# azuxmioy/Render-In-Between

Hardware: AMD Instinct MI355X
Metric: rendered frames/sec at 512x512 (generator forward + blend, device-resident) (higher is better)
Workload: dtype f32

## Files before the change

### include/rib.h

```cpp
#ifndef RIB_H
#define RIB_H

#include <stddef.h>
#include <stdint.h>

#ifdef __cplusplus
extern "C" {
#endif

typedef struct rib_handle rib_handle;

typedef enum {
  RIB_OK = 0,
  RIB_ERR_INVALID = -1,
  RIB_ERR_UNSUPPORTED = -2,
  RIB_ERR_STATE = -3,
  RIB_ERR_MISSING = -4,
  RIB_ERR_HIP = -5,
  RIB_ERR_WORKSPACE = -6
} rib_status;

typedef struct {
  int32_t label_nc;
  int32_t image_nc;
// ... 104 lines not shown
int rib_num_launches(rib_handle* h, int B, int H, int W);

int rib_num_variants(void);
int rib_variant_info(int idx, int geom[12]);
int rib_set_choice(rib_handle* h, int B, int H, int W, const char* op_name, int variant_idx, int ksplit);
int rib_time_op(rib_handle* h, int B, int H, int W, const char* op_name, const float* label,
                const float* img_fake, const float* img_prev, float* img, float* mask, void* workspace,
                size_t workspace_bytes, int iters, void* hip_stream, double* usec);

int rib_set_graph_replay(rib_handle* h, int enable);
int rib_graph_stats(rib_handle* h, int64_t* captures, int64_t* replays);

int rib_set_plan_batch(rib_handle* h, int n);
int rib_get_plan_batch(const rib_handle* h);

const char* rib_build_info(void);

int rib_debug_conv_weight(rib_handle* h, const char* conv_name, float* w_oihw, float* bias);
int rib_debug_spade_weight(rib_handle* h, const char* conv_name, float* w_2c_by_cond, float* bias_2c);
int rib_debug_launch_info(rib_handle* h, int B, int H, int W, int idx, char* buf, size_t buflen);

#ifdef __cplusplus
}
#endif
#endif
```

### render-in-between_amd/_native.py

```python
from __future__ import annotations

import ctypes as C
import os

_HERE = os.path.dirname(os.path.abspath(__file__))
LIB_PATH = os.environ.get("RIB_LIBRARY") or os.path.join(_HERE, "csrc", "librib.so")

KC_NAMES = ("igemm", "spade", "stats", "pool", "eltwise", "pack", "conv_aux")


class RibConfig(C.Structure):
    _fields_ = [(n, C.c_int32) for n in (
        "label_nc", "image_nc", "num_filters", "max_num_filters", "num_layers", "num_down_img",
        "emb_filters", "emb_max_filters", "emb_down", "mask_filters", "mask_max_filters",
        "mask_down", "mask_res_blocks")]


class RibError(RuntimeError):
    def __init__(self, code, msg):
        super().__init__("rib error %d: %s" % (code, msg))
        self.code = code


_lib = None
# ... 54 lines not shown
    "rib_forward_flops": (C.c_int, [C.c_void_p, C.c_int, C.c_int, C.c_int, C.POINTER(C.c_double)]),
    "rib_num_launches": (C.c_int, [C.c_void_p, C.c_int, C.c_int, C.c_int]),
    "rib_num_variants": (C.c_int, []),
    "rib_variant_info": (C.c_int, [C.c_int, C.POINTER(C.c_int)]),
    "rib_set_choice": (C.c_int, [C.c_void_p, C.c_int, C.c_int, C.c_int, C.c_char_p, C.c_int, C.c_int]),
    "rib_time_op": (C.c_int, [C.c_void_p, C.c_int, C.c_int, C.c_int, C.c_char_p] + [C.c_void_p] * 6
                    + [C.c_size_t, C.c_int, C.c_void_p, C.POINTER(C.c_double)]),
    "rib_debug_conv_weight": (C.c_int, [C.c_void_p, C.c_char_p, C.c_void_p, C.c_void_p]),
    "rib_debug_spade_weight": (C.c_int, [C.c_void_p, C.c_char_p, C.c_void_p, C.c_void_p]),
    "rib_debug_launch_info": (C.c_int, [C.c_void_p, C.c_int, C.c_int, C.c_int, C.c_int, C.c_char_p, C.c_size_t]),
    "rib_build_info": (C.c_char_p, []),
    "rib_set_graph_replay": (C.c_int, [C.c_void_p, C.c_int]),
    "rib_graph_stats": (C.c_int, [C.c_void_p, C.POINTER(C.c_int64), C.POINTER(C.c_int64)]),
    "rib_set_plan_batch": (C.c_int, [C.c_void_p, C.c_int]),
    "rib_get_plan_batch": (C.c_int, [C.c_void_p]),
}


def lib():
    global _lib
    if _lib is None:
        if not os.path.exists(LIB_PATH):
            raise RuntimeError(
                "native library %s is missing: build it with "
                "`python render-in-between_amd/csrc/build.py` (there is no CPU fallback)" % LIB_PATH)
        import torch
        L = C.CDLL(LIB_PATH)
        for name, (res, args) in SIGNATURES.items():
            fn = getattr(L, name)
            fn.restype = res
# ... 17 lines not shown
```

### render-in-between_amd/csrc/kernels.hip.h

```cpp
#pragma once
#include "igemm.hip.h"

namespace rib {

struct GemmDmaParams {
  const float* A; const float* B; float* C;
  int M, N, K, lda, ldc;
  size_t sA, sB, sC;
  int modB;
  int K2; unsigned long long kmask;
};

typedef uint32_t u32x4 __attribute__((ext_vector_type(4)));
__device__ __forceinline__ void split3_bf16(const float4 p, const float4 q, bf16x8& hi, bf16x8& mid, bf16x8& lo) {
  const float x[8] = {p.x, p.y, p.z, p.w, q.x, q.y, q.z, q.w};
  u32x4 h, m, l;
#pragma unroll
  for (int i = 0; i < 4; ++i) {
    const uint32_t u0 = __float_as_uint(x[2 * i]), u1 = __float_as_uint(x[2 * i + 1]);
    h[i] = __builtin_amdgcn_perm(u1, u0, 0x07060302u);
    const float r0 = x[2 * i] - __uint_as_float(u0 & 0xffff0000u), r1 = x[2 * i + 1] - __uint_as_float(u1 & 0xffff0000u);
    const uint32_t v0 = __float_as_uint(r0), v1 = __float_as_uint(r1);
    m[i] = __builtin_amdgcn_perm(v1, v0, 0x07060302u);
    const float s0 = r0 - __uint_as_float(v0 & 0xffff0000u), s1 = r1 - __uint_as_float(v1 & 0xffff0000u);
// ... 294 lines not shown
    for (int k = 0; k < 4; ++k) { t1 += red[(k * 64 + j) * 2]; t2 += red[(k * 64 + j) * 2 + 1]; }
    float sc, sh;
    scale_shift_of(t1, t2, s.inv_count, s.gamma ? s.gamma[c0 + j] : 1.f, s.beta ? s.beta[c0 + j] : 0.f, sc, sh);
    s_sc[j] = sc; s_sh[j] = sh;
  }
  __syncthreads();
}

enum { WSRC_PLAIN = 0, WSRC_SPADE = 1, WSRC_JOIN = 2 };
struct WinoInParams {
  const float* x; int H, W, xC, Cin;
  const float* pro_scale; const float* pro_shift; int pro_ld, pro_lrelu;
  StatSrc st;
  float* v; int tilesY, tilesX;
  int nslices, ublocks;
  int x_ups; const float* slab; int slab_ld, col0; const float* sbias;
  const float* x2; const float* xres; float* o; const float* pro2_scale; const float* pro2_shift; StatSrc st2;
  int ldv;
  int nslices2, Cin2, xC2, x2_ups, lrelu2, pro2_ld;
  const float* slab2; int slab2_ld, col0_2; const float* sbias2;
};
__device__ __forceinline__ WinoInParams wino_second(const WinoInParams& p) {
  WinoInParams q = p;
  q.x = p.x2; q.xC = p.xC2; q.Cin = p.Cin2; q.x_ups = p.x2_ups; q.pro_lrelu = p.lrelu2;
  q.pro_scale = p.pro2_scale; q.pro_shift = p.pro2_shift; q.pro_ld = p.pro2_ld; q.st = p.st2;
  q.slab = p.slab2; q.slab_ld = p.slab2_ld; q.col0 = p.col0_2; q.sbias = p.sbias2;
  q.x2 = nullptr; q.v = p.v + p.Cin;
  return q;
}

// ... 66 lines not shown
                    spade_mod1(r.a.z, k.sc.z, k.sh.z, r.b.z, k.bg.z, r.c.z, k.bb.z), spade_mod1(r.a.w, k.sc.w, k.sh.w, r.b.w, k.bg.w, r.c.w, k.bb.w));
    if (p.pro_lrelu) w = lrelu4(w);
  } else if constexpr (MODE == WSRC_JOIN) {
    w = make_float4(w.x * k.sc.x + k.sh.x, w.y * k.sc.y + k.sh.y, w.z * k.sc.z + k.sh.z, w.w * k.sc.w + k.sh.w);
    if (p.x2) { w.x += r.b.x * k.sc2.x + k.sh2.x; w.y += r.b.y * k.sc2.y + k.sh2.y; w.z += r.b.z * k.sc2.z + k.sh2.z; w.w += r.b.w * k.sc2.w + k.sh2.w; }
    else { w.x += r.b.x; w.y += r.b.y; w.z += r.b.z; w.w += r.b.w; }
  } else {
    if (k.aff) w = make_float4(w.x * k.sc.x + k.sh.x, w.y * k.sc.y + k.sh.y, w.z * k.sc.z + k.sh.z, w.w * k.sc.w + k.sh.w);
    if (p.pro_lrelu) w = lrelu4(w);
  }
  return w;
}

#define RIB_F4_SUB(a, b) make_float4((a).x - (b).x, (a).y - (b).y, (a).z - (b).z, (a).w - (b).w)
#define RIB_F4_ADD(a, b) make_float4((a).x + (b).x, (a).y + (b).y, (a).z + (b).z, (a).w + (b).w)

template <int MODE, bool SC>
__device__ __forceinline__ void wino_in_slice(const WinoInParams& p, int slice, int ub, double* red, float* s_sc, float* s_sh) {
  const int c4n = p.Cin / 4;
  const int n = blockIdx.y;
  const int c4 = slice * 16 + (threadIdx.x & 15);
  const bool cok = c4 < c4n;
  const int ntiles = p.tilesY * p.tilesX;
  constexpr int NR = SC ? 2 : 4, Q0 = SC ? 1 : 0, Q1 = SC ? 3 : 4;
  WinoConsts<MODE> kc;
  wino_in_consts<MODE>(p, n, slice, c4, cok, red, s_sc, s_sh, kc);
  if (!cok) return;
  for (int u = ub * 16 + (threadIdx.x >> 4); u < ntiles * NR; u += p.ublocks * 16) {
    const int r = SC ? 1 + (u & 1) : u & 3, tile = SC ? u >> 1 : u >> 2;
    const int ty = tile / p.tilesX, tx = tile % p.tilesX;
// ... 13 lines not shown
      float4 v[2];
#pragma unroll
      for (int a = 0; a < 2; ++a) {
        const int iy = 2 * ty - 1 + (a ? ib : ia), ix = 2 * tx - 1 + q;
        const bool inb = iy >= 0 && iy < p.H && ix >= 0 && ix < p.W;
        float4 w = wino_value<MODE>(p, kc, d[a][q]);
        if constexpr (MODE == WSRC_JOIN) {
          if (r == 1 && (q == 1 || q == 2) && inb) *reinterpret_cast<float4*>(p.o + (((size_t)n * p.H + iy) * p.W + ix) * p.xC + c4 * 4) = w;
        }
        if (!inb) w = make_float4(0.f, 0.f, 0.f, 0.f);
        v[a] = w;
      }
      t[q] = make_float4(v[0].x + sg * v[1].x, v[0].y + sg * v[1].y, v[0].z + sg * v[1].z, v[0].w + sg * v[1].w);
    }
    const size_t plane = (size_t)ntiles * p.ldv;
    float* vb = p.v + (size_t)n * 16 * plane + (size_t)tile * p.ldv + c4 * 4;
    if constexpr (!SC) *reinterpret_cast<float4*>(vb + (size_t)(r * 4 + 0) * plane) = RIB_F4_SUB(t[0], t[2]);
    *reinterpret_cast<float4*>(vb + (size_t)(r * 4 + 1) * plane) = RIB_F4_ADD(t[1], t[2]);
    *reinterpret_cast<float4*>(vb + (size_t)(r * 4 + 2) * plane) = RIB_F4_SUB(t[2], t[1]);
    if constexpr (!SC) *reinterpret_cast<float4*>(vb + (size_t)(r * 4 + 3) * plane) = RIB_F4_SUB(t[1], t[3]);
  }
}

template <int MODE, int MODE2 = -1>
__global__ __launch_bounds__(256) void k_wino_in(const WinoInParams p) {
  __shared__ double red[4 * 64 * 2];
  __shared__ float s_sc[64], s_sh[64];
  const int slice = blockIdx.x % p.nslices, ub = blockIdx.x / p.nslices;
  if constexpr (MODE2 >= 0) {
    const int n1 = p.nslices - p.nslices2;
    if (slice >= n1) { wino_in_slice<MODE2, true>(wino_second(p), slice - n1, ub, red, s_sc, s_sh); return; }
  }
  wino_in_slice<MODE, false>(p, slice, ub, red, s_sc, s_sh);
}

// ... 83 lines not shown
  if (p.stat_part) wino_out_partials(red, s1, s2, p.stat_part, n, p.ublocks, ub, slice, p.CoutPad);
}

__device__ __constant__ float kWino4BT[6][6] = {
    {81.f / 64, 0.f, -45.f / 16, 0.f, 1.f, 0.f},        {0.f, -27.f / 16, -9.f / 4, 3.f / 4, 1.f, 0.f},
    {0.f, 27.f / 16, -9.f / 4, -3.f / 4, 1.f, 0.f},     {0.f, -27.f / 32, -9.f / 16, 3.f / 2, 1.f, 0.f},
    {0.f, 27.f / 32, -9.f / 16, -3.f / 2, 1.f, 0.f},    {0.f, 81.f / 64, 0.f, -45.f / 16, 0.f, 1.f}};
__device__ __constant__ float kWino4AT[4][6] = {
    {1.f, 1.f, 1.f, 1.f, 1.f, 0.f},                      {0.f, 3.f / 4, -3.f / 4, 3.f / 2, -3.f / 2, 0.f},
    {0.f, 9.f / 16, 9.f / 16, 9.f / 4, 9.f / 4, 0.f},    {0.f, 27.f / 64, -27.f / 64, 27.f / 8, -27.f / 8, 1.f}};

__device__ __forceinline__ float4 f4_fma(float a, float4 x, float4 acc) {
  return make_float4(fmaf(a, x.x, acc.x), fmaf(a, x.y, acc.y), fmaf(a, x.z, acc.z), fmaf(a, x.w, acc.w));
}
__device__ __forceinline__ float4 f4_scale(float a, float4 x) { return make_float4(a * x.x, a * x.y, a * x.z, a * x.w); }

template <int MODE, bool SC>
__device__ __forceinline__ void wino4_in_slice(const WinoInParams& p, int slice, int ub, double* red, float* s_sc, float* s_sh) {
  const int c4n = p.Cin / 4;
  const int n = blockIdx.y;
  const int c4 = slice * 16 + (threadIdx.x & 15);
  const bool cok = c4 < c4n;
  const int ntiles = p.tilesY * p.tilesX;
  constexpr int NR = SC ? 4 : 6, Q0 = SC ? 1 : 0, Q1 = SC ? 5 : 6;
  WinoConsts<MODE> kc;
  wino_in_consts<MODE>(p, n, slice, c4, cok, red, s_sc, s_sh, kc);
  if (!cok) return;
  for (int u = ub * 16 + (threadIdx.x >> 4); u < ntiles * NR; u += p.ublocks * 16) {
    const int r = SC ? 1 + u % 4 : u % 6, tile = u / NR;
    const int ty = tile / p.tilesX, tx = tile % p.tilesX;
// ... 34 lines not shown
        for (int q = Q0; q < Q1; ++q) wino_fetch<MODE>(p, n, min(max(iy, 0), p.H - 1), min(max(4 * tx - 1 + q, 0), p.W - 1), c4, d[q]);
#pragma unroll
        for (int q = Q0; q < Q1; ++q) {
          const int ix = 4 * tx - 1 + q;
          const bool inb = iy >= 0 && iy < p.H && ix >= 0 && ix < p.W;
          float4 w = wino_value<MODE>(p, kc, d[q]);
          if constexpr (MODE == WSRC_JOIN) {
            if (r == 1 && q >= 1 && q <= 4 && inb) *reinterpret_cast<float4*>(p.o + (((size_t)n * p.H + iy) * p.W + ix) * p.xC + c4 * 4) = w;
          }
          if (!inb) w = make_float4(0.f, 0.f, 0.f, 0.f);
          t[q] = f4_fma(coef, w, t[q]);
        }
      }
    }
    const size_t plane = (size_t)ntiles * p.ldv;
    float* vb = p.v + (size_t)n * 36 * plane + (size_t)tile * p.ldv + c4 * 4;
    const float4 ev1 = f4_fma(-9.f / 4, t[2], t[4]), od1 = f4_fma(-27.f / 16, t[1], f4_scale(3.f / 4, t[3]));
    const float4 ev2 = f4_fma(-9.f / 16, t[2], t[4]), od2 = f4_fma(-27.f / 32, t[1], f4_scale(3.f / 2, t[3]));
    if constexpr (!SC) {
      const float4 e24 = f4_fma(-45.f / 16, t[2], t[4]);
      const float4 o13 = f4_fma(-45.f / 16, t[3], t[5]);
      *reinterpret_cast<float4*>(vb + (size_t)(r * 6 + 0) * plane) = f4_fma(81.f / 64, t[0], e24);
      *reinterpret_cast<float4*>(vb + (size_t)(r * 6 + 5) * plane) = f4_fma(81.f / 64, t[1], o13);
    }
    *reinterpret_cast<float4*>(vb + (size_t)(r * 6 + 1) * plane) = RIB_F4_ADD(ev1, od1);
    *reinterpret_cast<float4*>(vb + (size_t)(r * 6 + 2) * plane) = RIB_F4_SUB(ev1, od1);
    *reinterpret_cast<float4*>(vb + (size_t)(r * 6 + 3) * plane) = RIB_F4_ADD(ev2, od2);
    *reinterpret_cast<float4*>(vb + (size_t)(r * 6 + 4) * plane) = RIB_F4_SUB(ev2, od2);
  }
}

template <int MODE, int MODE2 = -1>
__global__ __launch_bounds__(256) void k_wino4_in(const WinoInParams p) {
  __shared__ double red[4 * 64 * 2];
  __shared__ float s_sc[64], s_sh[64];
  const int slice = blockIdx.x % p.nslices, ub = blockIdx.x / p.nslices;
  if constexpr (MODE2 >= 0) {
    const int n1 = p.nslices - p.nslices2;
    if (slice >= n1) { wino4_in_slice<MODE2, true>(wino_second(p), slice - n1, ub, red, s_sc, s_sh); return; }
  }
  wino4_in_slice<MODE, false>(p, slice, ub, red, s_sc, s_sh);
}

__global__ __launch_bounds__(256) void k_wino4_out(const WinoOutParams p) {
  __shared__ __attribute__((aligned(16))) double red[2][256][4];
  const int c4n = p.CoutPad / 4;
  const int slice = blockIdx.x % p.nslices, ub = blockIdx.x / p.nslices;
  const int c4 = slice * 16 + (threadIdx.x & 15);
  const int n = blockIdx.y;
  const int ntiles = p.tilesY * p.tilesX;
  double s1[4] = {0.0, 0.0, 0.0, 0.0}, s2[4] = {0.0, 0.0, 0.0, 0.0};
  if (c4 < c4n) {
    const float4 bv = *reinterpret_cast<const float4*>(p.bias + c4 * 4);
    const size_t plane = (size_t)ntiles * p.CoutPad;
    for (int unit = ub * 16 + (threadIdx.x >> 4); unit < ntiles * 4; unit += p.ublocks * 16) {
      const int tile = unit >> 2, r = unit & 3;
// ... 679 lines not shown
```

### render-in-between_amd/csrc/rib.hip

```cpp
#include "kernels.hip.h"
#include "rib_host.h"
#include <hip/hip_ext.h>

#include <algorithm>
#include <array>
#include <climits>
#include <cmath>
#include <cstdio>
#include <cstdlib>
#include <cstring>
#include <map>
#include <memory>
#include <string>
#include <variant>
#include <vector>


#include "variants.hip.h"
#define RIB_V(sec, ...) RIB_I_V(RIB_F_EXTERN, __VA_ARGS__)
#define RIB_VK(sec, ...) RIB_I_VK(RIB_F_EXTERN, __VA_ARGS__)
#define RIB_VT(sec, ...) RIB_I_VT(RIB_F_EXTERN, __VA_ARGS__)
#define RIB_VTK(sec, ...) RIB_I_VTK(RIB_F_EXTERN, __VA_ARGS__)
#define RIB_V9(sec, ...) RIB_I_V9(RIB_F_EXTERN, __VA_ARGS__)
#define RIB_VU4(sec, ...) RIB_I_VU4(RIB_F_EXTERN, __VA_ARGS__)
// ... 383 lines not shown
struct Op {
  int kclass = 0;
  std::string name;
  std::string for_op;
  bool label_only = false;
  dim3 grid;
  double flops = 0;
  const Variant* var = nullptr;
  int small_co = 0;
  bool head = false;
  bool fuse_blend = false;
  bool wino = false;
  int wino_m = 0;
  int wi_mode = 0;
  int wi_mode2 = -1;
  int lowc_ce = 0, lowc_ncol = 0, lowc_tw = 32;
  OpParams params;
  struct Binding { PRef ref; unsigned field = 0; };
  static constexpr int kMaxBindings = 24;
  Binding binds[kMaxBindings];
  int nbinds = 0;

  OpKind kind() const { return (OpKind)params.index(); }
  template <class P> const P& as() const { return std::get<P>(params); }
  template <class P, class T> unsigned field_of(T* P::*f) const {
    return (unsigned)(reinterpret_cast<const char*>(&(as<P>().*f)) - reinterpret_cast<const char*>(&params));
  }
  template <class P, class T> unsigned field_of(StatSrc P::*s, T* StatSrc::*f) const {
    return (unsigned)(reinterpret_cast<const char*>(&((as<P>().*s).*f)) - reinterpret_cast<const char*>(&params));
  }
// ... 79 lines not shown
  size_t d_blob_floats = 0;
  std::vector<float> host_blob;
  size_t blob_floats = 0;
  size_t zero_off = 0;
  uint64_t layout_hash = 0;
  struct WinoSet { int conv = 0, wm = 0; float* d = nullptr; size_t floats = 0; int aux = -1; };
  std::vector<WinoSet> wino_sets;
  std::map<std::array<int, 3>, int> wino_index;
  bool weights_ready = false;
  int prec_mode = PREC_F32;
  int prec() const { return prec_mode; }
  int products = 0;
  bool mc16() const { return prec_mode != PREC_F32; }
  int padc(int c) const { return mc16() ? pad16(c) : pad8(c); }
  int esz() const { return mc16() ? 2 : 4; }
  bool keep_taps = false;
  int plan_batch = 0;
  std::map<std::array<int, 5>, std::unique_ptr<Plan>> plans;
  std::map<std::string, std::pair<int, int>> choices;
  struct ChainGraph { std::array<uintptr_t, 12> key; hipGraphExec_t exec; uint64_t used; hipStream_t stream; };
  std::vector<ChainGraph> chain_graphs;
  bool graph_replay = false;
  uint64_t graph_clock = 0, graph_captures = 0, graph_replays = 0;
  bool profiling = false;
  bool prof_kernels = false;
  std::vector<std::pair<int, hipEvent_t>> prof_events;
  struct KernelEv { int kclass; hipEvent_t start, stop; };
  std::vector<KernelEv> prof_kernel_events;
  int64_t prof_launches[RIB_KC_COUNT] = {0};
  double prof_ms[RIB_KC_COUNT] = {0};
// ... 103 lines not shown
  }
  return RIB_OK;
}
void free_wino_sets(rib_handle* h) {
  for (auto& ws : h->wino_sets) if (ws.d) (void)hipFree(ws.d);
  h->wino_sets.clear(); h->wino_index.clear();
}

static bool lowc_instantiated(int ce, int ncol) {
  return (ce == 6 && ncol == 64) || (ce == 10 && ncol == 32) || (ce == 22 && ncol == 32) || (ce == 24 && ncol == 16);
}
template <int CE, int NCOL> static void launch_lowc_t(int tw, dim3 grid, hipStream_t st, const LowcParams& p) {
  if (tw == 16) RIB_KLAUNCH((k_conv_lowc<CE, NCOL, ST_F32, 16>), grid, dim3(256), 0, st, p);
  else RIB_KLAUNCH((k_conv_lowc<CE, NCOL, ST_F32, 32>), grid, dim3(256), 0, st, p);
}
static void launch_lowc(int ce, int ncol, int tw, dim3 grid, hipStream_t st, const LowcParams& p) {
  if (ce == 6 && ncol == 64) launch_lowc_t<6, 64>(tw, grid, st, p);
  else if (ce == 10 && ncol == 32) launch_lowc_t<10, 32>(tw, grid, st, p);
  else if (ce == 22 && ncol == 32) launch_lowc_t<22, 32>(tw, grid, st, p);
  else if (ce == 24 && ncol == 16) launch_lowc_t<24, 16>(tw, grid, st, p);
}

enum { BLOB_HEADER_FLOATS = 64, BLOB_MAGIC = 0x57424952 , BLOB_VERSION = 3 };
struct BlobHeader { uint32_t magic, version, prec, reserved; uint64_t floats, layout_hash; };

void assign_weight_layout(rib_handle* h) {
  size_t off = BLOB_HEADER_FLOATS;
  h->spades.clear(); h->spade_index.clear();
  auto take = [&](size_t nfloats) { size_t o = off; off += (nfloats + 63) / 64 * 64; return o; };
  h->zero_off = take(64);
// ... 501 lines not shown
      if (a.aux) {
        if (op.wi_mode == WSRC_JOIN) { error = gname + ": a join cannot carry a second source"; return false; }
        wi.nslices2 = (K2 + 63) / 64; wi.Cin2 = K2; wi.xC2 = a.aux_in.Cp;
        op.wi_mode2 = WSRC_PLAIN;
        if (a.aux_in.lazy) {
          const LazySrc& L = *a.aux_in.lazy;
          if (L.mode != WSRC_SPADE) { error = gname + ": lazy shortcut input of an unknown kind"; return false; }
          op.wi_mode2 = WSRC_SPADE;
          op.bind(&WinoInParams::x2, WS(L.x.off)); wi.xC2 = L.x.Cp; wi.pro2_ld = L.nx.ld; wi.x2_ups = L.x_ups ? 1 : 0; wi.lrelu2 = L.lrelu ? 1 : 0;
          if (!take_partials(L.nx, op, &WinoInParams::st2)) { materialize(L.nx, gname); op.bind(&WinoInParams::pro2_scale, WS(L.nx.sc)); op.bind(&WinoInParams::pro2_shift, WS(L.nx.sh)); }
          op.bind(&WinoInParams::slab2, WS(L.slab_off)); wi.slab2_ld = L.slab_ld; wi.col0_2 = L.col0; op.bind(&WinoInParams::sbias2, WT(L.sbias_off));
        } else op.bind(&WinoInParams::x2, WS(a.aux_in.off));
      }
      const int nsl = (c.cinp + 63) / 64 + wi.nslices2, units = ntiles * (wm + 2);
      wi.nslices = nsl; wi.ublocks = std::max(1, std::min((units + 15) / 16, (wi.st.tiles > 0 ? 512 : 4096) / nsl));
      op.grid = dim3(wi.ublocks * nsl, B, 1);
      push(op);
    }
    {
      Choice ch;
      ch.v = pick_gemm_dma(h->prec(), (long)TB_() * NP, ntiles, c.coutp, c.cinp);
      if (!ch.v) ch = choose_variant(h->prec(), 1, 1, false, false, c.coutp, TB_() * NP, tilesY, tilesX, c.cinp, false, 0, false);
      auto it = h->choices.find(fmt("%d,%d,%d|%s", TB_(), P->H, P->W, gname.c_str()));
      if (it != h->choices.end()) {
        const Variant& tv = kVariants[it->second.first];
        if (tv.BF16 != h->prec() || tv.KS != 1 || tv.STRIDE != 1 || tv.UPS || tv.SPADE || tv.NF == 0 || c.cinp % tv.BK != 0 || it->second.second != 1 || (a.aux && !tv.dma())) {
          error = fmt("%s: tuned choice (variant %d, ksplit %d) does not fit this layer", gname.c_str(), it->second.first, it->second.second); return false;
        }
        ch.v = &tv; ch.ksplit = 1;
      }
// ... 765 lines not shown
        } else
        RIB_KLAUNCH(pick_igemm_fn(op.var, p), op.grid, dim3(256 * op.var->KW), 0, st, p);
      } break;
      case OP_GEMM:
        RIB_KLAUNCH(h->products == RIB_PRODUCTS_BF16X3 && op.var->gfn_x3 ? op.var->gfn_x3 : op.var->gfn, op.grid, dim3(256), 0, st, std::get<GemmDmaParams>(params));
        break;
      case OP_FINALIZE: {
        const FinalizeParams& p = std::get<FinalizeParams>(params);
        if (p.tiles > 512) RIB_KLAUNCH(k_stats_finalize<4>, dim3((p.Cs + 3) / 4, op.grid.y, op.grid.z), dim3(1024), 0, st, p);
        else RIB_KLAUNCH(k_stats_finalize<16>, op.grid, dim3(1024), 0, st, p);
      } break;
      case OP_MODULATE: RIB_LAUNCH_ST(bf16, k_spade_modulate, op.grid, dim3(256), 0, st, std::get<ModulateParams>(params)); break;
      case OP_SPLITEPI: RIB_LAUNCH_ST(bf16, k_splitk_epilogue, op.grid, dim3(256), 0, st, std::get<SplitEpiParams>(params)); break;
      case OP_POOL: RIB_LAUNCH_ST(bf16, k_avgpool, op.grid, dim3(256), 0, st, std::get<PoolParams>(params)); break;
      case OP_INADD: RIB_LAUNCH_ST(bf16, k_in_add, op.grid, dim3(256), 0, st, std::get<InAddParams>(params)); break;
      case OP_WINO_IN: {
        const WinoInParams& p = std::get<WinoInParams>(params);
        if (op.wi_mode2 >= 0) {
          const bool s1 = op.wi_mode == WSRC_SPADE, s2 = op.wi_mode2 == WSRC_SPADE;
#define RIB_WINO_IN2(K)                                                                                     \
          if (s1 && s2) RIB_KLAUNCH((K<WSRC_SPADE, WSRC_SPADE>), op.grid, dim3(256), 0, st, p);             \
          else if (s1) RIB_KLAUNCH((K<WSRC_SPADE, WSRC_PLAIN>), op.grid, dim3(256), 0, st, p);              \
          else if (s2) RIB_KLAUNCH((K<WSRC_PLAIN, WSRC_SPADE>), op.grid, dim3(256), 0, st, p);              \
          else RIB_KLAUNCH((K<WSRC_PLAIN, WSRC_PLAIN>), op.grid, dim3(256), 0, st, p)
          if (op.wino_m == 4) { RIB_WINO_IN2(k_wino4_in); } else { RIB_WINO_IN2(k_wino_in); }
#undef RIB_WINO_IN2
        } else if (op.wino_m == 4) {
          if (op.wi_mode == WSRC_SPADE) RIB_KLAUNCH(k_wino4_in<WSRC_SPADE>, op.grid, dim3(256), 0, st, p);
          else if (op.wi_mode == WSRC_JOIN) RIB_KLAUNCH(k_wino4_in<WSRC_JOIN>, op.grid, dim3(256), 0, st, p);
          else RIB_KLAUNCH(k_wino4_in<WSRC_PLAIN>, op.grid, dim3(256), 0, st, p);
        } else {
          if (op.wi_mode == WSRC_SPADE) RIB_KLAUNCH(k_wino_in<WSRC_SPADE>, op.grid, dim3(256), 0, st, p);
          else if (op.wi_mode == WSRC_JOIN) RIB_KLAUNCH(k_wino_in<WSRC_JOIN>, op.grid, dim3(256), 0, st, p);
          else RIB_KLAUNCH(k_wino_in<WSRC_PLAIN>, op.grid, dim3(256), 0, st, p);
        }
      } break;
      case OP_WINO_OUT:
        if (op.wino_m == 4) RIB_KLAUNCH(k_wino4_out, op.grid, dim3(256), 0, st, std::get<WinoOutParams>(params));
        else RIB_KLAUNCH(k_wino_out, op.grid, dim3(256), 0, st, std::get<WinoOutParams>(params));
        break;
      case OP_LOWC: launch_lowc(op.lowc_ce, op.lowc_ncol, op.lowc_tw, op.grid, st, std::get<LowcParams>(params)); break;
      case OP_PACK: RIB_LAUNCH_ST(bf16, k_pack, op.grid, dim3(256), 0, st, std::get<PackParams>(params)); break;
    }
  }
  g_prof_pair = ProfPair();
  if (h->profiling && !h->prof_kernels) {
    hipEvent_t e1 = nullptr;
    HIP_TRY(h, hipEventCreate(&e1));
    HIP_TRY(h, hipEventRecord(e1, st));
    h->prof_events.push_back({-1, e1});
  }
// ... 11 lines not shown

extern "C" {

int rib_create(const rib_config* cfg, int device, rib_handle** out) {
  if (!cfg || !out) { g_create_error = "rib_create: null argument"; return RIB_ERR_INVALID; }
  *out = nullptr;
  const rib_config& c = *cfg;
  auto bad = [&](const std::string& m) { g_create_error = "rib_create: " + m; return RIB_ERR_UNSUPPORTED; };
  if (c.label_nc < 1 || c.image_nc < 1 || c.num_filters < 1 || c.num_down_img < 1 || c.mask_down < 1 ||
      c.emb_filters < 1 || c.mask_filters < 1 || c.mask_res_blocks < 1 || c.num_layers < c.num_down_img)
    return bad("invalid hyper-parameters");
  if (c.emb_down != c.num_down_img) return bad("embed.num_downsamples must equal num_downsamples_img (HSM.yaml: 4/4)");
  std::unique_ptr<rib_handle> h(new rib_handle());
  h->g.c = c; h->device = device; h->label_nc = c.label_nc;
  h->graph_replay = getenv("RIB_GRAPH") != nullptr && atoi(getenv("RIB_GRAPH")) != 0;
  for (int i = 0; i <= c.emb_down; ++i) {
    if (h->g.cond_ch(i) != h->g.emb_ch(i)) return bad("embed/generator max_num_filters disagree on the cond map width");
    if (h->g.emb_ch(i) % 32 != 0) return bad(fmt("embed width %d at level %d is not a multiple of 32", h->g.emb_ch(i), i));
  }
  for (int i = 1; i <= c.mask_down; ++i)
    if (h->g.mask_nf(i - 1) % 32 != 0) return bad("mask.num_filters must be a multiple of 32 (stride-2 kernels use 32-channel chunks)");
  for (int i = 0; i <= c.num_down_img + 1; ++i) {
    const int ch = h->g.nf(i);
    if (ch % 4 != 0 || 256 % (ch / 4 > 0 ? ch / 4 : 1) != 0 || ch > 1024) return bad(fmt("generator width %d unsupported (power-of-two multiples of 4 up to 1024)", ch));
  }
  h->convs = build_inventory(h->g);
  for (size_t i = 0; i < h->convs.size(); ++i) h->conv_index[h->convs[i].name] = (int)i;
  register_tensors(h.get());
  assign_weight_layout(h.get());
  if (device >= 0) {
// ... 445 lines not shown
      rc = rib_blend(h, B, c.image_nc, H, W, img_t, mask_t, dains + (size_t)t * frame, fuse_t, hip_stream);
      if (rc) return rc;
    }
    prev = fuse_t;
  }
  return RIB_OK;
}

int rib_set_debug_taps(rib_handle* h, int enable) {
  if (!h) return RIB_ERR_INVALID;
  if (h->keep_taps != (enable != 0)) { h->plans.clear(); drop_chain_graphs(h); }
  h->keep_taps = enable != 0;
  return RIB_OK;
}

int rib_num_taps(rib_handle* h, int B, int H, int W) {
  if (!h) return RIB_ERR_INVALID;
  Plan* P = get_plan(h, B, H, W);
  return P ? (int)P->taps.size() : RIB_ERR_INVALID;
}

int rib_tap_info(rib_handle* h, int B, int H, int W, int idx, const char** name, int* C, int* th, int* tw) {
  if (!h) return RIB_ERR_INVALID;
  Plan* P = get_plan(h, B, H, W);
  if (!P || idx < 0 || idx >= (int)P->taps.size()) return RIB_ERR_INVALID;
  const Tap& t = P->taps[idx];
  if (name) *name = t.name.c_str();
  if (C) *C = t.C;
  if (th) *th = t.H;
  if (tw) *tw = t.W;
// ... 58 lines not shown

static int launch_info_head(const Op& op, char* buf, size_t buflen) {
  if (op.kind() == OP_IGEMM && op.small_co > 0)
    snprintf(buf, buflen, "%s|%d|%u,%u,%u|%s 16x16 tile, %d output channels%s|%.0f", op.name.c_str(), op.kclass, op.grid.x, op.grid.y, op.grid.z,
             op.head ? "head (taps as MFMA columns)" : "direct (vector ALUs)", op.small_co, op.fuse_blend ? " + fused blend" : "", op.flops);
  else if (op.kind() == OP_IGEMM)
    snprintf(buf, buflen, "%s|%d|%u,%u,%u|tile %dx%d BN %d BK %d s%d k%d ups%d ksplit%d kw%d tb%d%s v%d|%.0f", op.name.c_str(), op.kclass, op.grid.x, op.grid.y, op.grid.z,
             op.var->TH(), op.var->TW(), op.var->BN(), op.var->BK, op.var->STRIDE, op.var->KS, (int)op.var->UPS, op.as<IgemmParams>().ksplit, op.var->KW, op.var->DMAK ? 100 + (op.var->TB == 9 ? 9 : 0) : op.var->TB,
             op.wino ? (op.wino_m == 4 ? " wino4" : " wino") : "", (int)(op.var - kVariants), op.flops);
  else if (op.kind() == OP_GEMM)
    snprintf(buf, buflen, "%s|%d|%u,%u,%u|gemm (LDS-DMA staged operands) tile %dx%d BK 32, %d x [%d x %d x %d]%s|%.0f", op.name.c_str(), op.kclass, op.grid.x, op.grid.y, op.grid.z,
             op.var->BM(), op.var->BN(), (int)op.grid.z, op.as<GemmDmaParams>().M, op.as<GemmDmaParams>().N, op.as<GemmDmaParams>().K, (std::string(op.wino ? (op.wino_m == 4 ? " wino4" : " wino") : "") + (op.as<GemmDmaParams>().K2 ? fmt(" + K %d of the 1x1 shortcut at %d positions", op.as<GemmDmaParams>().K2, __builtin_popcountll(op.as<GemmDmaParams>().kmask)) : std::string())).c_str(), op.flops);
  else if (op.kind() == OP_LOWC)
    snprintf(buf, buflen, "%s|%d|%u,%u,%u|lowc (caller's NCHW tensors, K = 9 x %d real channels) 8x%d tile, %d columns|%.0f", op.name.c_str(), op.kclass,
             op.grid.x, op.grid.y, op.grid.z, op.lowc_ce, op.lowc_tw, op.lowc_ncol, op.flops);
  else
    snprintf(buf, buflen, "%s|%d|%u,%u,%u||0", op.name.c_str(), op.kclass, op.grid.x, op.grid.y, op.grid.z);
  return RIB_OK;
}

static double op_algorithmic_bytes(const rib_handle* h, const Plan* P, const Op& op) {
  const double e = h->esz(), Bn = P->B;
  switch (op.kind()) {
    case OP_IGEMM: {
      const IgemmParams& p = op.as<IgemmParams>();
      const double samples = p.pair ? 2.0 * Bn : Bn;
      const int taps = op.var ? op.var->KS * op.var->KS : 9;
      double b = samples * p.Hin * p.Win * (double)p.Cin * e
                 + (double)p.CoutPad * taps * p.Cin * e * (p.pair ? 2.0 : 1.0)
                 + p.CoutPad * 4.0;
// ... 214 lines not shown
```

### render-in-between_amd/generator.py

```python
from __future__ import annotations

import ctypes as C
from typing import Dict, Optional

import torch

from . import _native
from .config import GenSpec


def _ptr(t: Optional[torch.Tensor]):
    return C.c_void_p(t.data_ptr()) if t is not None else C.c_void_p(0)


class Generator:
    def __init__(self, gen_cfg, device=None, use_tuning=True, compute_dtype="f32", products="f32"):
        if compute_dtype not in ("f32", "bf16", "f16"):
            raise ValueError("compute_dtype must be 'f32', 'bf16' or 'f16'")
        if products not in ("f32", "bf16x3"):
            raise ValueError("products must be 'f32' or 'bf16x3'")
        if products != "f32" and compute_dtype != "f32":
            raise ValueError("products='bf16x3' is an option of the fp32 mode")
        self.compute_dtype = compute_dtype
        self.products = products
# ... 246 lines not shown
                fz = torch.empty((T, B, s.image_nc, H, W), dtype=torch.float32, device=self.device)
                ring["sets"].append((torch.empty_like(fz) if want_all else None,
                                     torch.empty((T, B, 1, H, W), dtype=torch.float32, device=self.device) if want_all else None, fz))
            imgs, masks, fuses = ring["sets"][ring["n"] % len(ring["sets"])] if len(ring["sets"]) == 2 else ring["sets"][-1]
            ring["n"] += 1
        else:
            fuses = torch.empty((T, B, s.image_nc, H, W), dtype=torch.float32, device=self.device)
            imgs = torch.empty_like(fuses) if want_all else None
            masks = torch.empty((T, B, 1, H, W), dtype=torch.float32, device=self.device) if want_all else None
        with torch.cuda.device(self.device):
            _native.check(self._h, self._lib.rib_chain(
                self._h, T, B, H, W, _ptr(key_frame), _ptr(labels), _ptr(dains), _ptr(imgs), _ptr(masks),
                _ptr(fuses), _ptr(ws), ws.numel(), self._stream()))
        return imgs, masks, fuses

    def set_graph_replay(self, on=True):
        _native.check(self._h, self._lib.rib_set_graph_replay(self._h, 1 if on else 0))
        self._graph_replay = bool(on)
        self.__dict__.pop("_chain_out", None)
        return self

    def graph_stats(self):
        cap, rep = C.c_int64(), C.c_int64()
        _native.check(self._h, self._lib.rib_graph_stats(self._h, C.byref(cap), C.byref(rep)))
        return {"captures": cap.value, "replays": rep.value}

    def blend(self, img, mask, dain):
        img = img.to(self.device, torch.float32).contiguous(); mask = mask.to(self.device, torch.float32).contiguous()
        dain = dain.to(self.device, torch.float32).contiguous()
        B, Cc, H, W = img.shape
# ... 397 lines not shown
```

Baseline: 398.5.

## Stage Winograd input patches in LDS so overlapping tile halos are fetched once

Adds a staged Winograd input-transform kernel in which each workgroup loads a shared patch covering several adjacent tiles into LDS, then computes the B^T d B rows from that patch rather than re-fetching the overlapping halo pixels per tile. The planner enables it by default when the patch fits in a fixed pixel budget and enough workgroups remain, and an environment variable or API call turns it off. The aim is to cut redundant global reads and normalisation work in the input transform. In exchange it adds an LDS footprint and a barrier, and it reduces the number of workgroups, which may lower occupancy or parallelism on small layers.

Result: faster. 402.5 (median of 6 runs) (+1.0%).

```diff
diff --git a/include/rib.h b/include/rib.h
--- a/include/rib.h
+++ b/include/rib.h
@@ -142,6 +142,8 @@
 int rib_set_plan_batch(rib_handle* h, int n);
 int rib_get_plan_batch(const rib_handle* h);
 
+int rib_set_wino_in_staging(rib_handle* h, int on);
+
 const char* rib_build_info(void);
 
 int rib_debug_conv_weight(rib_handle* h, const char* conv_name, float* w_oihw, float* bias);
diff --git a/render-in-between_amd/_native.py b/render-in-between_amd/_native.py
--- a/render-in-between_amd/_native.py
+++ b/render-in-between_amd/_native.py
@@ -92,6 +92,7 @@
     "rib_graph_stats": (C.c_int, [C.c_void_p, C.POINTER(C.c_int64), C.POINTER(C.c_int64)]),
     "rib_set_plan_batch": (C.c_int, [C.c_void_p, C.c_int]),
     "rib_get_plan_batch": (C.c_int, [C.c_void_p]),
+    "rib_set_wino_in_staging": (C.c_int, [C.c_void_p, C.c_int]),
 }
 
 
diff --git a/render-in-between_amd/csrc/kernels.hip.h b/render-in-between_amd/csrc/kernels.hip.h
--- a/render-in-between_amd/csrc/kernels.hip.h
+++ b/render-in-between_amd/csrc/kernels.hip.h
@@ -332,6 +332,7 @@
   StatSrc st;
   float* v; int tilesY, tilesX;
   int nslices, ublocks;
+  int sty, stx;
   int x_ups; const float* slab; int slab_ld, col0; const float* sbias;
   const float* x2; const float* xres; float* o; const float* pro2_scale; const float* pro2_shift; StatSrc st2;
   int ldv;
@@ -428,6 +429,14 @@
 
 #define RIB_F4_SUB(a, b) make_float4((a).x - (b).x, (a).y - (b).y, (a).z - (b).z, (a).w - (b).w)
 #define RIB_F4_ADD(a, b) make_float4((a).x + (b).x, (a).y + (b).y, (a).z + (b).z, (a).w + (b).w)
+
+template <bool SC>
+__device__ __forceinline__ void wino_store_row(float* vb, size_t plane, int r, const float4 (&t)[4]) {
+  if constexpr (!SC) *reinterpret_cast<float4*>(vb + (size_t)(r * 4 + 0) * plane) = RIB_F4_SUB(t[0], t[2]);
+  *reinterpret_cast<float4*>(vb + (size_t)(r * 4 + 1) * plane) = RIB_F4_ADD(t[1], t[2]);
+  *reinterpret_cast<float4*>(vb + (size_t)(r * 4 + 2) * plane) = RIB_F4_SUB(t[2], t[1]);
+  if constexpr (!SC) *reinterpret_cast<float4*>(vb + (size_t)(r * 4 + 3) * plane) = RIB_F4_SUB(t[1], t[3]);
+}
 
 template <int MODE, bool SC>
 __device__ __forceinline__ void wino_in_slice(const WinoInParams& p, int slice, int ub, double* red, float* s_sc, float* s_sh) {
@@ -471,11 +480,7 @@
       t[q] = make_float4(v[0].x + sg * v[1].x, v[0].y + sg * v[1].y, v[0].z + sg * v[1].z, v[0].w + sg * v[1].w);
     }
     const size_t plane = (size_t)ntiles * p.ldv;
-    float* vb = p.v + (size_t)n * 16 * plane + (size_t)tile * p.ldv + c4 * 4;
-    if constexpr (!SC) *reinterpret_cast<float4*>(vb + (size_t)(r * 4 + 0) * plane) = RIB_F4_SUB(t[0], t[2]);
-    *reinterpret_cast<float4*>(vb + (size_t)(r * 4 + 1) * plane) = RIB_F4_ADD(t[1], t[2]);
-    *reinterpret_cast<float4*>(vb + (size_t)(r * 4 + 2) * plane) = RIB_F4_SUB(t[2], t[1]);
-    if constexpr (!SC) *reinterpret_cast<float4*>(vb + (size_t)(r * 4 + 3) * plane) = RIB_F4_SUB(t[1], t[3]);
+    wino_store_row<SC>(p.v + (size_t)n * 16 * plane + (size_t)tile * p.ldv + c4 * 4, plane, r, t);
   }
 }
 
@@ -589,6 +594,22 @@
   return make_float4(fmaf(a, x.x, acc.x), fmaf(a, x.y, acc.y), fmaf(a, x.z, acc.z), fmaf(a, x.w, acc.w));
 }
 __device__ __forceinline__ float4 f4_scale(float a, float4 x) { return make_float4(a * x.x, a * x.y, a * x.z, a * x.w); }
+
+template <bool SC>
+__device__ __forceinline__ void wino4_store_row(float* vb, size_t plane, int r, const float4 (&t)[6]) {
+  const float4 ev1 = f4_fma(-9.f / 4, t[2], t[4]), od1 = f4_fma(-27.f / 16, t[1], f4_scale(3.f / 4, t[3]));
+  const float4 ev2 = f4_fma(-9.f / 16, t[2], t[4]), od2 = f4_fma(-27.f / 32, t[1], f4_scale(3.f / 2, t[3]));
+  if constexpr (!SC) {
+    const float4 e24 = f4_fma(-45.f / 16, t[2], t[4]);
+    const float4 o13 = f4_fma(-45.f / 16, t[3], t[5]);
+    *reinterpret_cast<float4*>(vb + (size_t)(r * 6 + 0) * plane) = f4_fma(81.f / 64, t[0], e24);
+    *reinterpret_cast<float4*>(vb + (size_t)(r * 6 + 5) * plane) = f4_fma(81.f / 64, t[1], o13);
+  }
+  *reinterpret_cast<float4*>(vb + (size_t)(r * 6 + 1) * plane) = RIB_F4_ADD(ev1, od1);
+  *reinterpret_cast<float4*>(vb + (size_t)(r * 6 + 2) * plane) = RIB_F4_SUB(ev1, od1);
+  *reinterpret_cast<float4*>(vb + (size_t)(r * 6 + 3) * plane) = RIB_F4_ADD(ev2, od2);
+  *reinterpret_cast<float4*>(vb + (size_t)(r * 6 + 4) * plane) = RIB_F4_SUB(ev2, od2);
+}
 
 template <int MODE, bool SC>
 __device__ __forceinline__ void wino4_in_slice(const WinoInParams& p, int slice, int ub, double* red, float* s_sc, float* s_sh) {
@@ -653,19 +674,7 @@
       }
     }
     const size_t plane = (size_t)ntiles * p.ldv;
-    float* vb = p.v + (size_t)n * 36 * plane + (size_t)tile * p.ldv + c4 * 4;
-    const float4 ev1 = f4_fma(-9.f / 4, t[2], t[4]), od1 = f4_fma(-27.f / 16, t[1], f4_scale(3.f / 4, t[3]));
-    const float4 ev2 = f4_fma(-9.f / 16, t[2], t[4]), od2 = f4_fma(-27.f / 32, t[1], f4_scale(3.f / 2, t[3]));
-    if constexpr (!SC) {
-      const float4 e24 = f4_fma(-45.f / 16, t[2], t[4]);
-      const float4 o13 = f4_fma(-45.f / 16, t[3], t[5]);
-      *reinterpret_cast<float4*>(vb + (size_t)(r * 6 + 0) * plane) = f4_fma(81.f / 64, t[0], e24);
-      *reinterpret_cast<float4*>(vb + (size_t)(r * 6 + 5) * plane) = f4_fma(81.f / 64, t[1], o13);
-    }
-    *reinterpret_cast<float4*>(vb + (size_t)(r * 6 + 1) * plane) = RIB_F4_ADD(ev1, od1);
-    *reinterpret_cast<float4*>(vb + (size_t)(r * 6 + 2) * plane) = RIB_F4_SUB(ev1, od1);
-    *reinterpret_cast<float4*>(vb + (size_t)(r * 6 + 3) * plane) = RIB_F4_ADD(ev2, od2);
-    *reinterpret_cast<float4*>(vb + (size_t)(r * 6 + 4) * plane) = RIB_F4_SUB(ev2, od2);
+    wino4_store_row<SC>(p.v + (size_t)n * 36 * plane + (size_t)tile * p.ldv + c4 * 4, plane, r, t);
   }
 }
 
@@ -679,6 +688,99 @@
     if (slice >= n1) { wino4_in_slice<MODE2, true>(wino_second(p), slice - n1, ub, red, s_sc, s_sh); return; }
   }
   wino4_in_slice<MODE, false>(p, slice, ub, red, s_sc, s_sh);
+}
+
+constexpr int WINO_STAGE_MAX_PX = 100;
+constexpr int WINO_STAGE_LDS_BYTES = WINO_STAGE_MAX_PX * 64 * 4 + 4 * 64 * 2 * 8 + 2 * 64 * 4;
+
+template <int M, int MODE>
+__device__ __forceinline__ void wino_in_staged_slice(const WinoInParams& p, int slice, int blk, float4* patch, double* red, float* s_sc,
+                                                     float* s_sh) {
+  constexpr int NR = M + 2, NF = (WINO_STAGE_MAX_PX + 15) / 16;
+  const int n = blockIdx.y;
+  const int lane = threadIdx.x & 15, slot = threadIdx.x >> 4;
+  const int c4 = slice * 16 + lane;
+  const bool cok = c4 < p.Cin / 4;
+  const int nbx = (p.tilesX + p.stx - 1) / p.stx;
+  const int ty0 = (blk / nbx) * p.sty, tx0 = (blk % nbx) * p.stx;
+  const int ph = M * p.sty + 2, pw = M * p.stx + 2, npix = ph * pw;
+  const int y0 = M * ty0 - 1, x0 = M * tx0 - 1;
+  WinoRaw<MODE> d[NF];
+#pragma unroll
+  for (int i = 0; i < NF; ++i) {
+    const int pi = i * 16 + slot;
+    if (cok && pi < npix) wino_fetch<MODE>(p, n, min(max(y0 + pi / pw, 0), p.H - 1), min(max(x0 + pi % pw, 0), p.W - 1), c4, d[i]);
+  }
+  WinoConsts<MODE> kc;
+  wino_in_consts<MODE>(p, n, slice, c4, cok, red, s_sc, s_sh, kc);
+#pragma unroll
+  for (int i = 0; i < NF; ++i) {
+    const int pi = i * 16 + slot;
+    if (cok && pi < npix) {
+      const int py = pi / pw, px = pi % pw, iy = y0 + py, ix = x0 + px;
+      const bool inb = iy >= 0 && iy < p.H && ix >= 0 && ix < p.W;
+      float4 w = wino_value<MODE>(p, kc, d[i]);
+      if constexpr (MODE == WSRC_JOIN) {
+        if (inb && py >= 1 && py < ph - 1 && px >= 1 && px < pw - 1) *reinterpret_cast<float4*>(p.o + (((size_t)n * p.H + iy) * p.W + ix) * p.xC + c4 * 4) = w;
+      }
+      if (!inb) w = make_float4(0.f, 0.f, 0.f, 0.f);
+      patch[pi * 16 + lane] = w;
+    }
+  }
+  __syncthreads();
+  if (!cok) return;
+  const int ntiles = p.tilesY * p.tilesX;
+  const size_t plane = (size_t)ntiles * p.ldv;
+  for (int u = slot; u < p.sty * p.stx * NR; u += 16) {
+    const int r = u % NR, tl = u / NR, tyl = tl / p.stx, txl = tl % p.stx;
+    const int ty = ty0 + tyl, tx = tx0 + txl;
+    if (ty >= p.tilesY || tx >= p.tilesX) continue;
+    const float4* d0 = patch + ((M * tyl) * pw + M * txl) * 16 + lane;
+    float* vb = p.v + (size_t)n * (NR * NR) * plane + (size_t)(ty * p.tilesX + tx) * p.ldv + c4 * 4;
+    if constexpr (M == 2) {
+      const int ia = r == 0 ? 0 : (r == 2 ? 2 : 1), ib = r == 0 ? 2 : (r == 1 ? 2 : (r == 2 ? 1 : 3));
+      const float sg = r == 1 ? 1.f : -1.f;
+      float4 t[4];
+#pragma unroll
+      for (int q = 0; q < 4; ++q) {
+        const float4 v0 = d0[(ia * pw + q) * 16], v1 = d0[(ib * pw + q) * 16];
+        t[q] = make_float4(v0.x + sg * v1.x, v0.y + sg * v1.y, v0.z + sg * v1.z, v0.w + sg * v1.w);
+      }
+      wino_store_row<false>(vb, plane, r, t);
+    } else {
+      const int a0 = r == 0 ? 0 : 1, da = (r == 0 || r == 5) ? 2 : 1, na = (r == 0 || r == 5) ? 3 : 4;
+      float4 t[6];
+#pragma unroll
+      for (int q = 0; q < 6; ++q) t[q] = make_float4(0.f, 0.f, 0.f, 0.f);
+#pragma unroll
+      for (int k = 0; k < 4; ++k) {
+        if (MODE != WSRC_PLAIN && k >= na) break;
+        const int a = a0 + min(k, na - 1) * da;
+        const float coef = k < na ? kWino4BT[r][a] : 0.f;
+#pragma unroll
+        for (int q = 0; q < 6; ++q) t[q] = f4_fma(coef, d0[(a * pw + q) * 16], t[q]);
+      }
+      wino4_store_row<false>(vb, plane, r, t);
+    }
+  }
+}
+
+template <int M, int MODE, int MODE2 = -1>
+__global__ __launch_bounds__(256) void k_wino_in_staged(const WinoInParams p) {
+  __shared__ float4 patch[WINO_STAGE_MAX_PX * 16];
+  __shared__ double red[4 * 64 * 2];
+  __shared__ float s_sc[64], s_sh[64];
+  static_assert(sizeof(patch) + sizeof(red) + sizeof(s_sc) + sizeof(s_sh) == WINO_STAGE_LDS_BYTES, "the planner's figure");
+  const int slice = blockIdx.x % p.nslices, blk = blockIdx.x / p.nslices;
+  if constexpr (MODE2 >= 0) {
+    const int n1 = p.nslices - p.nslices2;
+    if (slice >= n1) {
+      if constexpr (M == 4) wino4_in_slice<MODE2, true>(wino_second(p), slice - n1, blk, red, s_sc, s_sh);
+      else wino_in_slice<MODE2, true>(wino_second(p), slice - n1, blk, red, s_sc, s_sh);
+      return;
+    }
+  }
+  wino_in_staged_slice<M, MODE>(p, slice, blk, patch, red, s_sc, s_sh);
 }
 
 __global__ __launch_bounds__(256) void k_wino4_out(const WinoOutParams p) {
diff --git a/render-in-between_amd/csrc/rib.hip b/render-in-between_amd/csrc/rib.hip
--- a/render-in-between_amd/csrc/rib.hip
+++ b/render-in-between_amd/csrc/rib.hip
@@ -421,6 +421,7 @@
   int wino_m = 0;
   int wi_mode = 0;
   int wi_mode2 = -1;
+  bool wi_staged = false;
   int lowc_ce = 0, lowc_ncol = 0, lowc_tw = 32;
   OpParams params;
   struct Binding { PRef ref; unsigned field = 0; };
@@ -530,6 +531,7 @@
   bool mc16() const { return prec_mode != PREC_F32; }
   int padc(int c) const { return mc16() ? pad16(c) : pad8(c); }
   int esz() const { return mc16() ? 2 : 4; }
+  bool wino_in_staging = true;
   bool keep_taps = false;
   int plan_batch = 0;
   std::map<std::array<int, 5>, std::unique_ptr<Plan>> plans;
@@ -663,6 +665,23 @@
   if (tw == 16) RIB_KLAUNCH((k_conv_lowc<CE, NCOL, ST_F32, 16>), grid, dim3(256), 0, st, p);
   else RIB_KLAUNCH((k_conv_lowc<CE, NCOL, ST_F32, 32>), grid, dim3(256), 0, st, p);
 }
+template <int M, bool STAGED, int MODE, int MODE2 = -1> static void launch_wino_in_t(dim3 grid, hipStream_t st, const WinoInParams& p) {
+  if constexpr (STAGED) RIB_KLAUNCH((k_wino_in_staged<M, MODE, MODE2>), grid, dim3(256), 0, st, p);
+  else if constexpr (M == 4) RIB_KLAUNCH((k_wino4_in<MODE, MODE2>), grid, dim3(256), 0, st, p);
+  else RIB_KLAUNCH((k_wino_in<MODE, MODE2>), grid, dim3(256), 0, st, p);
+}
+template <int M, bool STAGED> static void launch_wino_in(const Op& op, hipStream_t st, const WinoInParams& p) {
+  if (op.wi_mode2 >= 0) {
+    const bool s1 = op.wi_mode == WSRC_SPADE, s2 = op.wi_mode2 == WSRC_SPADE;
+    if (s1 && s2) launch_wino_in_t<M, STAGED, WSRC_SPADE, WSRC_SPADE>(op.grid, st, p);
+    else if (s1) launch_wino_in_t<M, STAGED, WSRC_SPADE, WSRC_PLAIN>(op.grid, st, p);
+    else if (s2) launch_wino_in_t<M, STAGED, WSRC_PLAIN, WSRC_SPADE>(op.grid, st, p);
+    else launch_wino_in_t<M, STAGED, WSRC_PLAIN, WSRC_PLAIN>(op.grid, st, p);
+  } else if (op.wi_mode == WSRC_SPADE) launch_wino_in_t<M, STAGED, WSRC_SPADE>(op.grid, st, p);
+  else if (op.wi_mode == WSRC_JOIN) launch_wino_in_t<M, STAGED, WSRC_JOIN>(op.grid, st, p);
+  else launch_wino_in_t<M, STAGED, WSRC_PLAIN>(op.grid, st, p);
+}
+
 static void launch_lowc(int ce, int ncol, int tw, dim3 grid, hipStream_t st, const LowcParams& p) {
   if (ce == 6 && ncol == 64) launch_lowc_t<6, 64>(tw, grid, st, p);
   else if (ce == 10 && ncol == 32) launch_lowc_t<10, 32>(tw, grid, st, p);
@@ -1194,6 +1213,17 @@
       }
       const int nsl = (c.cinp + 63) / 64 + wi.nslices2, units = ntiles * (wm + 2);
       wi.nslices = nsl; wi.ublocks = std::max(1, std::min((units + 15) / 16, (wi.st.tiles > 0 ? 512 : 4096) / nsl));
+      if (h->wino_in_staging) {
+        static const int kBlocks2[][2] = {{4, 4}, {2, 4}, {2, 2}}, kBlocks4[][2] = {{2, 2}, {1, 2}, {1, 1}};
+        const int need = std::min((int)(wi.ublocks * nsl * B), 256 );
+        const bool fits = 2 * WINO_STAGE_LDS_BYTES <= 160 * 1024 ;
+        for (int i = 0; i < 3 && fits && !op.wi_staged; ++i) {
+          const int sty = std::min((wm == 4 ? kBlocks4 : kBlocks2)[i][0], tilesY), stx = std::min((wm == 4 ? kBlocks4 : kBlocks2)[i][1], tilesX);
+          const int nblocks = ((tilesY + sty - 1) / sty) * ((tilesX + stx - 1) / stx);
+          if ((wm * sty + 2) * (wm * stx + 2) > WINO_STAGE_MAX_PX || nblocks * nsl * B < need) continue;
+          op.wi_staged = true; wi.sty = sty; wi.stx = stx; wi.ublocks = nblocks;
+        }
+      }
       op.grid = dim3(wi.ublocks * nsl, B, 1);
       push(op);
     }
@@ -1989,27 +2019,10 @@
       case OP_SPLITEPI: RIB_LAUNCH_ST(bf16, k_splitk_epilogue, op.grid, dim3(256), 0, st, std::get<SplitEpiParams>(params)); break;
       case OP_POOL: RIB_LAUNCH_ST(bf16, k_avgpool, op.grid, dim3(256), 0, st, std::get<PoolParams>(params)); break;
       case OP_INADD: RIB_LAUNCH_ST(bf16, k_in_add, op.grid, dim3(256), 0, st, std::get<InAddParams>(params)); break;
-      case OP_WINO_IN: {
-        const WinoInParams& p = std::get<WinoInParams>(params);
-        if (op.wi_mode2 >= 0) {
-          const bool s1 = op.wi_mode == WSRC_SPADE, s2 = op.wi_mode2 == WSRC_SPADE;
-#define RIB_WINO_IN2(K)                                                                                     \
-          if (s1 && s2) RIB_KLAUNCH((K<WSRC_SPADE, WSRC_SPADE>), op.grid, dim3(256), 0, st, p);             \
-          else if (s1) RIB_KLAUNCH((K<WSRC_SPADE, WSRC_PLAIN>), op.grid, dim3(256), 0, st, p);              \
-          else if (s2) RIB_KLAUNCH((K<WSRC_PLAIN, WSRC_SPADE>), op.grid, dim3(256), 0, st, p);              \
-          else RIB_KLAUNCH((K<WSRC_PLAIN, WSRC_PLAIN>), op.grid, dim3(256), 0, st, p)
-          if (op.wino_m == 4) { RIB_WINO_IN2(k_wino4_in); } else { RIB_WINO_IN2(k_wino_in); }
-#undef RIB_WINO_IN2
-        } else if (op.wino_m == 4) {
-          if (op.wi_mode == WSRC_SPADE) RIB_KLAUNCH(k_wino4_in<WSRC_SPADE>, op.grid, dim3(256), 0, st, p);
-          else if (op.wi_mode == WSRC_JOIN) RIB_KLAUNCH(k_wino4_in<WSRC_JOIN>, op.grid, dim3(256), 0, st, p);
-          else RIB_KLAUNCH(k_wino4_in<WSRC_PLAIN>, op.grid, dim3(256), 0, st, p);
-        } else {
-          if (op.wi_mode == WSRC_SPADE) RIB_KLAUNCH(k_wino_in<WSRC_SPADE>, op.grid, dim3(256), 0, st, p);
-          else if (op.wi_mode == WSRC_JOIN) RIB_KLAUNCH(k_wino_in<WSRC_JOIN>, op.grid, dim3(256), 0, st, p);
-          else RIB_KLAUNCH(k_wino_in<WSRC_PLAIN>, op.grid, dim3(256), 0, st, p);
-        }
-      } break;
+      case OP_WINO_IN:
+        if (op.wino_m == 4) { if (op.wi_staged) launch_wino_in<4, true>(op, st, std::get<WinoInParams>(params)); else launch_wino_in<4, false>(op, st, std::get<WinoInParams>(params)); }
+        else { if (op.wi_staged) launch_wino_in<2, true>(op, st, std::get<WinoInParams>(params)); else launch_wino_in<2, false>(op, st, std::get<WinoInParams>(params)); }
+        break;
       case OP_WINO_OUT:
         if (op.wino_m == 4) RIB_KLAUNCH(k_wino4_out, op.grid, dim3(256), 0, st, std::get<WinoOutParams>(params));
         else RIB_KLAUNCH(k_wino_out, op.grid, dim3(256), 0, st, std::get<WinoOutParams>(params));
@@ -2051,6 +2064,7 @@
   std::unique_ptr<rib_handle> h(new rib_handle());
   h->g.c = c; h->device = device; h->label_nc = c.label_nc;
   h->graph_replay = getenv("RIB_GRAPH") != nullptr && atoi(getenv("RIB_GRAPH")) != 0;
+  h->wino_in_staging = !(getenv("RIB_WINO_IN_UNSTAGED") != nullptr && atoi(getenv("RIB_WINO_IN_UNSTAGED")) != 0);
   for (int i = 0; i <= c.emb_down; ++i) {
     if (h->g.cond_ch(i) != h->g.emb_ch(i)) return bad("embed/generator max_num_filters disagree on the cond map width");
     if (h->g.emb_ch(i) % 32 != 0) return bad(fmt("embed width %d at level %d is not a multiple of 32", h->g.emb_ch(i), i));
@@ -2526,6 +2540,13 @@
   return RIB_OK;
 }
 
+int rib_set_wino_in_staging(rib_handle* h, int on) {
+  if (!h) return RIB_ERR_INVALID;
+  if (h->wino_in_staging != (on != 0)) { h->plans.clear(); drop_chain_graphs(h); }
+  h->wino_in_staging = on != 0;
+  return RIB_OK;
+}
+
 int rib_num_taps(rib_handle* h, int B, int H, int W) {
   if (!h) return RIB_ERR_INVALID;
   Plan* P = get_plan(h, B, H, W);
@@ -2614,6 +2635,9 @@
   else if (op.kind() == OP_LOWC)
     snprintf(buf, buflen, "%s|%d|%u,%u,%u|lowc (caller's NCHW tensors, K = 9 x %d real channels) 8x%d tile, %d columns|%.0f", op.name.c_str(), op.kclass,
              op.grid.x, op.grid.y, op.grid.z, op.lowc_ce, op.lowc_tw, op.lowc_ncol, op.flops);
+  else if (op.kind() == OP_WINO_IN && op.wi_staged)
+    snprintf(buf, buflen, "%s|%d|%u,%u,%u|staged, %dx%d tiles per workgroup|0", op.name.c_str(), op.kclass, op.grid.x, op.grid.y, op.grid.z,
+             op.as<WinoInParams>().sty, op.as<WinoInParams>().stx);
   else
     snprintf(buf, buflen, "%s|%d|%u,%u,%u||0", op.name.c_str(), op.kclass, op.grid.x, op.grid.y, op.grid.z);
   return RIB_OK;
diff --git a/render-in-between_amd/generator.py b/render-in-between_amd/generator.py
--- a/render-in-between_amd/generator.py
+++ b/render-in-between_amd/generator.py
@@ -284,6 +284,10 @@
                 _ptr(fuses), _ptr(ws), ws.numel(), self._stream()))
         return imgs, masks, fuses
 
+    def set_wino_in_staging(self, on=True):
+        _native.check(self._h, self._lib.rib_set_wino_in_staging(self._h, 1 if on else 0))
+        return self
+
     def set_graph_replay(self, on=True):
         _native.check(self._h, self._lib.rib_set_graph_replay(self._h, 1 if on else 0))
         self._graph_replay = bool(on)
```
